# fluggo/Canvas

Measured on AMD Instinct MI355X. Metric: Mpixels/s through 4K f16 RGBA colour-matrix+alpha-over chain; % HBM roofline, higher is better.
Workload: dtype f32

## Files before the change

### canvas_amd/_lib.py

```python
import ctypes as C
import os

from .abi import (box2i, fir_filter, rational, rgba_frame_f16, rgba_frame_f32, v2f, v2i, video_frame_source_funcs,
                  video_source)

_HERE = os.path.dirname(os.path.abspath(__file__))
LIB_PATH = os.path.join(_HERE, "libcanvas_hip.so")

CHAIN_MAX_LAYERS = 8
DISPLAY_RGBA8, DISPLAY_ARGB32_PREMUL = 0, 1
FIR_PATH_AUTO, FIR_PATH_PASSES, FIR_PATH_TILED, FIR_PATH_TABLES, FIR_PATH_HV, FIR_PATH_ONE_COLUMN, FIR_PATH_TWO_COLUMNS, FIR_PATH_STRIPS, FIR_PATH_TILES = 0, 1, 2, 4, 16, 32, 64, 128, 256
FIR_KERNEL_NONE, FIR_KERNEL_WINDOW, FIR_KERNEL_HALVE, _FIR_KERNEL_RETIRED_3, FIR_KERNEL_VH, FIR_KERNEL_TILED, _FIR_KERNEL_RETIRED_6, FIR_KERNEL_TWO_PASS, FIR_KERNEL_PASS, FIR_KERNEL_HV, FIR_KERNEL_WINDOW_PAIR, FIR_KERNEL_HALVE_PAIR, FIR_KERNEL_TILE_VH, FIR_KERNEL_UNSHARP = range(14)
ARITH_SEPARATE, ARITH_CONTRACTED = 0, 1
LUT_NONE, LUT_REC709_TO_LINEAR_SCENE, LUT_REC709_TO_LINEAR_DISPLAY, LUT_LINEAR_TO_REC709, LUT_LINEAR_TO_SRGB = -1, 0, 1, 2, 3
KEY_SHOW_MATTE = 1
MATTE_SHOW, MATTE_MAX_CHOKE, MATTE_MAX_TAPS = 1, 16, 25
TRANSFORM_NEAREST, TRANSFORM_BILINEAR, TRANSFORM_MAX_COORD = 0, 1, 1 << 23
MAX_COORD, RESAMPLE_MAX_COORD = 1 << 30, 1 << 23
SCOPE_HISTOGRAM, SCOPE_WAVEFORM, SCOPE_PARADE, SCOPE_VECTORSCOPE = range(4)
SCOPE_SKIP_TRANSPARENT, SCOPE_MAX_COLUMNS = 1, 4096
LUT3D_MIN_SIZE, LUT3D_MAX_SIZE = 2, 65
PERSPECTIVE_MAX_SPAN = 1 << 23
YCC_PROGRESSIVE, YCC_REC709 = 1, 2

# ... 233 lines not shown
    "cvs_transform_from_parts": (C.c_int, [P(C.c_double), P(C.c_double), C.c_double, P(C.c_double), _f32p]),
    "cvs_transform_target_window": (C.c_int, [P(transform_params), P(box2i), P(box2i), P(box2i)]),
    "cvs_transform_source_window": (C.c_int, [P(transform_params), P(box2i), P(box2i)]),
    "cvs_blur_over_f16_dev": (C.c_int, [_F16, _F16, _f32p, C.c_int, P(_F16), C.c_int, _vp]),
    "cvs_resample_lanczos_f32_dev": (C.c_int, [_F32, _F32, C.c_float, C.c_float, C.c_int, _vp]),
    "cvs_resample_lanczos_f16_dev": (C.c_int, [_F16, _F16, C.c_float, C.c_float, C.c_int, _vp]),
    "cvs_blur_lanczos_f16_dev": (C.c_int, [_F16, _F16, _f32p, C.c_int, C.c_float, C.c_float, C.c_int, _vp]),
    "cvs_blur_over_f16_batch_dev": (C.c_int, [P(_F16), P(_F16), _f32p, C.c_int, P(_F16), C.c_int, C.c_int, _vp]),
    "cvs_scale_bilinear_f16_batch_dev": (C.c_int, [P(_F16), v2f, P(_F16), v2f, v2f, C.c_int, _vp]),
    "cvs_scale_bilinear_f32_batch_dev": (C.c_int, [P(_F32), v2f, P(_F32), v2f, v2f, C.c_int, _vp]),
    "cvs_blur_lanczos_f16_batch_dev": (C.c_int, [P(_F16), P(_F16), C.c_int, _f32p, C.c_int, C.c_float, C.c_float, C.c_int, _vp]),
    "cvs_fir_path_override": (None, [C.c_int]),
    "cvs_chain_color_over_f16_dev": (C.c_int, [P(chain_job), C.c_int, _f32p, C.c_int, C.c_int, _vp]),
    "cvs_chain_last_was_fused": (C.c_int, []),
    "cvs_scale_last_was_fused": (C.c_int, []),
    "cvs_fir_last_kernel": (C.c_int, []),
    "cvs_fir_fell_through_count": (C.c_int, []),
    "cvs_chain_last_launch_count": (C.c_int, []),
    "cvs_mix_cross_f16_dev": (C.c_int, [_F16, _F16, _F16, C.c_float, _vp]),
}

SCOPE_SIGNATURES = {
    "cvs_scope_count": (C.c_size_t, [P(scope_params)]),
    "cvs_scope_picture_size": (C.c_int, [P(scope_params), P(v2i)]),
    "cvs_scope_counts_f16_dev": (C.c_int, [_vp, _F16, P(scope_params), _vp]),
    "cvs_scope_render_f16_dev": (C.c_int, [_F16, P(box2i), _vp, P(scope_params), C.c_float, _vp]),
    "video_scope_counts": (C.c_int, [_vp, _F16, P(scope_params)]),
}

LUT3D_SIGNATURES = {
    "cvs_lut3d_bytes": (C.c_size_t, [C.c_int]),
    "cvs_lut3d_pack": (C.c_int, [_f32p, _f32p, C.c_int]),
    "cvs_lut3d_f16_dev": (C.c_int, [_F16, _F16, _vp, P(lut3d_params), _vp]),
    "cvs_lut3d_f32_dev": (C.c_int, [_F32, _F32, _vp, P(lut3d_params), _vp]),
}

PERSPECTIVE_SIGNATURES = {
    "cvs_perspective_f32_dev": (C.c_int, [_F32, _F32, P(perspective_params), _vp]),
    "cvs_perspective_f16_dev": (C.c_int, [_F16, _F16, P(perspective_params), _vp]),
    "cvs_perspective_from_quad": (C.c_int, [P(C.c_double), P(C.c_double * 2), C.c_int, P(perspective_params)]),
    "cvs_perspective_target_window": (C.c_int, [P(perspective_params), P(box2i), P(box2i), P(box2i)]),
    "cvs_perspective_source_window": (C.c_int, [P(perspective_params), P(box2i), P(box2i)]),
}

DEINTERLACE_SIGNATURES = {
    "cvs_deinterlace_adaptive_f16_dev": (C.c_int, [_F16, _F16, _F16, _F16, P(deinterlace_params), _vp]),
}

MEDIAN_SIGNATURES = {
    "cvs_median_f16_dev": (C.c_int, [_F16, _F16, P(median_params), _vp]),
    "cvs_median_f32_dev": (C.c_int, [_F32, _F32, P(median_params), _vp]),
}

HALF_POINTER_GLOBALS = {
    "half_convert_to_float": C.CFUNCTYPE(None, _f32p, _u16p, C.c_int),
    "half_convert_from_float": C.CFUNCTYPE(None, _u16p, _f32p, C.c_int),
    "half_convert_to_float_fast": C.CFUNCTYPE(None, _f32p, _u16p, C.c_int),
    "half_convert_from_float_fast": C.CFUNCTYPE(None, _u16p, _f32p, C.c_int),
    "half_lookup": C.CFUNCTYPE(None, _u16p, _u16p, _u16p, C.c_int),
}

_lib = None


class LibraryMissing(RuntimeError):
    pass


def load():
    global _lib
    if _lib is not None:
        return _lib
    if not os.path.exists(LIB_PATH):
        raise LibraryMissing(
            "%s not found: build it with `python -c 'import __graft_entry__ as g; g.build()'` "
            "(or make -C canvas_amd/csrc).  There is no CPU fallback." % LIB_PATH)
    lib = C.CDLL(LIB_PATH, mode=C.RTLD_GLOBAL)
    for name, (res, args) in list(SIGNATURES.items()) + list(SCOPE_SIGNATURES.items()) + list(LUT3D_SIGNATURES.items()) + list(PERSPECTIVE_SIGNATURES.items()) + list(DEINTERLACE_SIGNATURES.items()) + list(MEDIAN_SIGNATURES.items()):
        fn = getattr(lib, name)
        fn.restype, fn.argtypes = res, args
    _lib = lib
    return lib


def half_pointer(name):
    lib = load()
    addr = C.c_void_p.in_dll(lib, name).value
    return HALF_POINTER_GLOBALS[name](addr) if addr else None


def last_error():
    return load().cvs_last_error().decode()


def check(rc, what="call"):
    if rc != 0:
        raise RuntimeError("%s failed (%d): %s" % (what, rc, last_error()))
```

### canvas_amd/csrc/host/scale.c

```c
#define _GNU_SOURCE
#include "internal.h"
#include <limits.h>
#include <math.h>
#include <stdatomic.h>

static _Atomic int g_fir_path = CVS_FIR_PATH_AUTO;

static _Thread_local int t_scale_fused;
CVS_EXPORT int cvs_scale_last_was_fused(void) { return t_scale_fused; }
static _Thread_local int t_fir_kernel;
CVS_EXPORT int cvs_fir_last_kernel(void) { return t_fir_kernel; }
static _Thread_local int t_fell_through;
CVS_EXPORT int cvs_fir_fell_through_count(void) { return t_fell_through; }
static void fir_launch_fell_through(const char *kernel, int rc) {
    (void)hipGetLastError();
    t_fell_through++;
    cvs_log_warning("%s did not launch (%s): falling back to the next FIR kernel", kernel, hipGetErrorString((hipError_t)rc));
}
CVS_EXPORT void cvs_fir_path_override(int mode) { atomic_store(&g_fir_path, mode & (CVS_FIR_PATH_PASSES | CVS_FIR_PATH_TILED | CVS_FIR_PATH_TABLES | CVS_FIR_PATH_HV | CVS_FIR_PATH_ONE_COLUMN | CVS_FIR_PATH_TWO_COLUMNS | CVS_FIR_PATH_STRIPS | CVS_FIR_PATH_TILES)); }

typedef struct { void *data; box2i full, cur; int half; } any_frame;

static size_t any_bytes(const any_frame *f) { return cvs_box_pixels(&f->full) * (f->half ? sizeof(rgba_f16) : sizeof(rgba_f32)); }

typedef struct { void *frame, *data; box2i *full, *cur; } frame_ref;

static frame_ref frame_of(const void *f, int half) {
    frame_ref r = { (void *)f, NULL, NULL, NULL };
    if (f && half) { rgba_frame_f16 *h = r.frame; r.data = h->data; r.full = &h->full_window; r.cur = &h->current_window; }
    else if (f)    { rgba_frame_f32 *g = r.frame; r.data = g->data; r.full = &g->full_window; r.cur = &g->current_window; }
    return r;
}

static frame_ref frame_at(const void *frames, int i, int half) {
    return frame_of(half ? (const void *)((const rgba_frame_f16 *const *)frames)[i] : (const void *)((const rgba_frame_f32 *const *)frames)[i], half);
}

static any_frame any_of(const frame_ref *f, int half) {
    const any_frame a = { f->data, *f->full, *f->cur, half };
    return a;
}

static bool shares_buffer(const frame_ref *t, const frame_ref *src, const char *what) {
    if (!t->data || t->data != src->data) return false;
    cvs_set_error("%s: the target is the source's buffer: the operation is not in place", what);
    return true;
}

static bool entry_refused(void *target, const void *source, int half, const char *what, frame_ref *t, frame_ref *src, int lim) {
    *t = frame_of(target, half);
    *src = frame_of(source, half);
    if (shares_buffer(t, src, what)) { box2i_set_empty(t->cur); return true; }
    if (cvs_enter() != 0) { box2i_set_empty(t->cur); return true; }
    if (!cvs_box_contains(src->full, src->cur)) {
// ... 662 lines not shown
        else box2i_set_empty(&target->current_window);
        return rc;
    }
    any_frame mid = { NULL, *sw, *sw, 0 };
    mid.data = cvs_pool_malloc(cvs_box_pixels(sw) * sizeof(rgba_f32), s);
    if (!mid.data) { box2i_set_empty(&target->current_window); return -1; }
    int rc = blur_fused(&mid, &sf, sw, taps, ntaps, NULL, 0, NULL, s);
    if (rc == 0) rc = lanczos_fused(&tf, &mid, fx, fy, ksize, s);
    if (rc == 0) target->current_window = target->full_window;
    cvs_pool_free(mid.data, s);
    if (rc != 0) box2i_set_empty(&target->current_window);
    return rc;
}

CVS_EXPORT int cvs_blur_over_f16_batch_dev(rgba_frame_f16 *const *outs, const rgba_frame_f16 *const *sources, const float *taps, int ntaps,
                                           const rgba_frame_f16 *const *overlays, int noverlays, int count, cvs_stream_t stream) {
    const char *what = "cvs_blur_over_f16_batch_dev";
    if (count <= 0) return 0;
    if (ntaps < 1 || !taps || noverlays < 0 || (noverlays > 0 && !overlays)) { cvs_set_error("%s: bad arguments", what); return -1; }
    for (int i = 0; i < count; i++)
        for (int l = 0; l < noverlays; l++)
            if (!overlays[(size_t)i * noverlays + l]) { cvs_set_error("%s: layer %d of frame %d is a null pointer", what, l, i); return -1; }
    if (batch_refused(outs, sources, count, 1, what, CVS_MAX_COORD)) return -1;
    for (int i = 0; i < count * noverlays; i++)
        if (cvs_coords_refused(what, "an overlay", &overlays[i]->full_window, &overlays[i]->current_window, CVS_MAX_COORD)) { batch_empty_from(outs, 0, count, 1); return -1; }
    hipStream_t s = cvs_pick_stream(stream);
    const box2i *full = &outs[0]->full_window;
    bool uniform = count > 1 && noverlays >= 1 && noverlays <= CVK_BLUR_MAX_OVER && !box2i_is_empty(full) && blur_has_fast_kernel(taps, ntaps) && (ntaps & 1);
    for (int i = 0; uniform && i < count; i++) {
        uniform = same_box(&outs[i]->full_window, full) && same_box(&sources[i]->full_window, &sources[0]->full_window) &&
                  same_box(&sources[i]->current_window, full) && same_box(&sources[0]->full_window, full);
        for (int l = 0; uniform && l < noverlays; l++) {
            const rgba_frame_f16 *ov = overlays[(size_t)i * noverlays + l];
            uniform = same_box(&ov->full_window, full) && same_box(&ov->current_window, full);
        }
    }
    int rc = 0, done = 0;
    const size_t bytes = cvs_box_pixels(full) * sizeof(rgba_f16);
    while (uniform && rc == 0 && done < count) {
        const int n = count - done < CVK_FRAME_BATCH ? count - done : CVK_FRAME_BATCH;
        cvk_frame_batch b;
        if (!batch_group(&b, outs, sources, 1, done, n, bytes, bytes, overlays, noverlays)) break;
        const any_frame t = { b.target[0], *full, *full, 1 }, src = { (void *)b.source[0], sources[done]->full_window, sources[done]->current_window, 1 };
        rc = blur_fused(&t, &src, full, taps, ntaps, b.over[0], noverlays, &b, s);
        if (rc == 1) { rc = 0; break; }
        if (rc == 0) { for (int i = 0; i < n; i++) outs[done + i]->current_window = *full; done += n; }
    }
    for (; rc == 0 && done < count; done++)
        rc = cvs_blur_over_f16_dev(outs[done], sources[done], taps, ntaps, noverlays ? overlays + (size_t)done * noverlays : NULL, noverlays, stream);
    if (rc != 0) batch_empty_from(outs, done, count, 1);
    return rc;
}

CVS_EXPORT int cvs_blur_lanczos_f16_batch_dev(rgba_frame_f16 *const *targets, const rgba_frame_f16 *const *sources, int count,
                                              const float *taps, int ntaps, float fx, float fy, int ksize, cvs_stream_t stream) {
    const char *what = "cvs_blur_lanczos_f16_batch_dev";
    if (count <= 0) return 0;
    if (ntaps < 1 || !taps || !(fx > 0.0f) || !(fy > 0.0f) || ksize < 1) { cvs_set_error("%s: bad arguments", what); return -1; }
    if (batch_refused(targets, sources, count, 1, what, CVS_RESAMPLE_MAX_COORD)) return -1;
    hipStream_t s = cvs_pick_stream(stream);
    int rc = 0, done = 0;
    const box2i *tf = &targets[0]->full_window, *sw = &sources[0]->current_window;
    bool uniform = count > 1 && (ntaps & 1) && !(ntaps == 1 && taps[0] == 1.0f) && !box2i_is_empty(sw) && !box2i_is_empty(tf);
    for (int i = 1; uniform && i < count; i++)
        uniform = same_box(&targets[i]->full_window, tf) && same_box(&sources[i]->full_window, &sources[0]->full_window) &&
                  same_box(&sources[i]->current_window, sw);
    const any_frame t0 = { targets[0]->data, *tf, *tf, 1 }, s0 = { (void *)sources[0]->data, sources[0]->full_window, *sw, 1 };
    cvk_blur_halve_params hp;
    if (uniform && halving_sweep(&hp, fx, fy, ksize, taps, ntaps, &t0, &s0) && CVK(cvk_blur_halve_supported)(ntaps, hp.ntaps2)) {
        const size_t sbytes = cvs_box_pixels(&sources[0]->full_window) * sizeof(rgba_f16), tbytes = cvs_box_pixels(tf) * sizeof(rgba_f16);
        while (rc == 0 && done < count) {
            const int n = count - done < CVK_FRAME_BATCH ? count - done : CVK_FRAME_BATCH;
            if (!batch_group(&hp.batch, targets, sources, 1, done, n, tbytes, sbytes, NULL, 0)) break;
            hp.target.data = hp.batch.target[0];
            hp.source.data = (void *)hp.batch.source[0];
            if ((rc = halving_launch(&hp, s)) != 0) break;
            for (int i = 0; i < n; i++) targets[done + i]->current_window = targets[done + i]->full_window;
            done += n;
        }
    }
    for (; rc == 0 && done < count; done++)
        rc = cvs_blur_lanczos_f16_dev(targets[done], sources[done], taps, ntaps, fx, fy, ksize, stream);
    if (rc != 0) batch_empty_from(targets, done, count, 1);
    return rc;
}
```

### canvas_amd/csrc/kernels/kernels.h

```cpp
#ifndef CVS_KERNELS_H
#define CVS_KERNELS_H

#include <stddef.h>
#include <stdint.h>

#ifdef CVS_DIAG
#include <stdlib.h>
#define CVS_DIAG_ENV(name) getenv(name)
#else
#define CVS_DIAG_ENV(name) ((const char *)0)
#endif

#ifdef CVS_CONTRACT
#define cvk_gain_offset_f16          cvk_gain_offset_f16_fma
#define cvk_mix                      cvk_mix_fma
#define cvk_color_matrix             cvk_color_matrix_fma
#define cvk_chain_color_over         cvk_chain_color_over_fma
#define cvk_chain_cross              cvk_chain_cross_fma
#define cvk_chain_count_reset        cvk_chain_count_reset_fma
#define cvk_chain_count              cvk_chain_count_fma
#define cvk_fir_gather               cvk_fir_gather_fma
#define cvk_fir2d_lds_bytes          cvk_fir2d_lds_bytes_fma
#define cvk_fir2d                    cvk_fir2d_fma
#define cvk_fir_vh_supported         cvk_fir_vh_supported_fma
#define cvk_fir_vh                   cvk_fir_vh_fma
#define cvk_fir_tvh_supported        cvk_fir_tvh_supported_fma
#define cvk_fir_tvh_preferred        cvk_fir_tvh_preferred_fma
#define cvk_fir_tvh                  cvk_fir_tvh_fma
#define cvk_blur_supported           cvk_blur_supported_fma
#define cvk_blur_takes_pairs         cvk_blur_takes_pairs_fma
#define cvk_blur                     cvk_blur_fma
#define cvk_blur_pair_supported      cvk_blur_pair_supported_fma
#define cvk_blur_pair                cvk_blur_pair_fma
#define cvk_blur_halve_pair_supported cvk_blur_halve_pair_supported_fma
#define cvk_blur_halve_pair          cvk_blur_halve_pair_fma
#define cvk_blur_halve_supported     cvk_blur_halve_supported_fma
#define cvk_blur_halve_takes_pairs   cvk_blur_halve_takes_pairs_fma
#define cvk_blur_halve               cvk_blur_halve_fma
#define cvk_unsharp_supported        cvk_unsharp_supported_fma
#define cvk_unsharp                  cvk_unsharp_fma
#define cvk_unsharp_combine          cvk_unsharp_combine_fma
#define cvk_dv_reconstruct           cvk_dv_reconstruct_fma
#define cvk_dv_subsample             cvk_dv_subsample_fma
#endif

#ifdef __cplusplus
extern "C" {
#endif

typedef struct {
    void *data;
    int pitch;
    int fx0, fy0, fx1, fy1;
} cvk_view;

typedef struct { int x0, y0, x1, y1; } cvk_rect;

int cvk_half_to_float(float *out, const uint16_t *in, size_t count, int fast, void *stream);
int cvk_float_to_half(uint16_t *out, const float *in, size_t count, int fast, void *stream);
int cvk_half_lookup(const uint16_t *table, uint16_t *out, const uint16_t *in, size_t count, int cus, void *stream);

int cvk_copy_f16(cvk_view out, cvk_view in, cvk_rect r, void *stream);
int cvk_copy_alpha_f32(cvk_view out, cvk_view in, cvk_rect r, float alpha, void *stream);
int cvk_weave_f16(cvk_view frame, cvk_rect cur, const void *other, cvk_rect other_cur, void *stream);
int cvk_widen(cvk_view out32, cvk_view in16, cvk_rect r, void *stream);
int cvk_narrow(cvk_view out16, cvk_view in32, cvk_rect r, void *stream);
int cvk_fill_f16(cvk_view out, cvk_rect r, const float rgba[4], void *stream);
int cvk_fill_f32(cvk_view out, cvk_rect r, const float rgba[4], void *stream);
int cvk_gain_offset_f16(cvk_view out, cvk_view in, cvk_rect r, float gain, float offset, void *stream);

enum { CVK_MIX_CROSS = 0, CVK_MIX_OVER = 1 };
typedef struct {
    cvk_view out, p, q;
    cvk_rect outer, inner;
    cvk_rect pw, qw;
    int gap_x, gap_y;
    int top_is_p, bottom_is_p, left_is_p, right_is_p;
    float wp, wq;
    int mode;
    int p_in_place;
} cvk_mix_params;
int cvk_mix(const cvk_mix_params *mp, void *stream);

int cvk_color_matrix(cvk_view dst, cvk_view src, cvk_rect r, const float m[9], const uint16_t *pre_lut,
                     const uint16_t *post_lut, int cus, void *stream);

// ... 52 lines not shown
#define CVK_FIR_TVH_LINES 16
typedef struct {
    cvk_view target, source;
    int in_half, out_half;
    int tx0, ty0, tx1, ty1;
    cvk_fir_axis h, v;
    int max_sw, max_sh;
    int nframes, pad_;
    const void *frame_source[8];
    void *frame_target[8];
} cvk_fir2d_params;
#define CVK_FIR2D_TILE_X 32
#define CVK_FIR2D_TILE_Y 16
int cvk_fir_hv_supported(const cvk_fir2d_params *fp);
int cvk_fir_hv(const cvk_fir2d_params *fp, int cus, void *stream);
int cvk_fir_vh_supported(const cvk_fir2d_params *fp);
int cvk_fir_vh(const cvk_fir2d_params *fp, int line0, int cus, void *stream);
int cvk_fir_tvh_supported(const cvk_fir2d_params *fp);
int cvk_fir_tvh_preferred(const cvk_fir2d_params *fp);
int cvk_fir_tvh(const cvk_fir2d_params *fp, int line0, void *stream);
size_t cvk_fir2d_lds_bytes(const cvk_fir2d_params *fp);
int cvk_fir2d(const cvk_fir2d_params *fp, void *stream);

#define CVK_FRAME_BATCH 8
#define CVK_BLUR_MAX_OVER 4
typedef struct {
    int n, pad;
    const void *source[CVK_FRAME_BATCH];
    void *target[CVK_FRAME_BATCH];
    const void *over[CVK_FRAME_BATCH][CVK_BLUR_MAX_OVER];
} cvk_frame_batch;

typedef struct {
    cvk_view target, source;
    int in_half, out_half;
    int tx0, ty0, tx1, ty1;
    int sx0, sy0, sx1, sy1;
    int ntaps;
    int rows_per_wg;
    int step;
    float taps[32];
    int nover;
    int flags;
    const void *over[CVK_BLUR_MAX_OVER];
    cvk_frame_batch batch;
} cvk_blur_params;
#define CVK_BLUR_ONE_COLUMN  1
#define CVK_BLUR_TWO_COLUMNS 2
int cvk_blur_supported(int ntaps, int step);
int cvk_blur(const cvk_blur_params *bp, int cus, void *stream);
int cvk_blur_takes_pairs(const cvk_blur_params *bp);
int cvk_blur_pair_supported(const cvk_blur_params *bp);
int cvk_blur_pair(const cvk_blur_params *bp, int cus, void *stream);

typedef struct {
    cvk_view target, source;
    int in_half, out_half;
    int tx0, ty0, tx1, ty1;
    int sx0, sy0, sx1, sy1;
    int ntaps1, ntaps2;
    int rows_per_wg;
    int flags;
    float taps1[16], taps2[16];
    cvk_frame_batch batch;
} cvk_blur_halve_params;
int cvk_blur_halve_supported(int ntaps1, int ntaps2);
int cvk_blur_halve_pair_supported(const cvk_blur_halve_params *bp);
int cvk_blur_halve_pair(const cvk_blur_halve_params *bp, int cus, void *stream);
int cvk_blur_halve_takes_pairs(const cvk_blur_halve_params *bp);
int cvk_blur_halve(const cvk_blur_halve_params *bp, int cus, void *stream);

typedef struct {
    cvk_view target, source;
    int half;
    int tx0, ty0, tx1, ty1;
    int sx0, sy0, sx1, sy1;
    int ntaps;
    int rows_per_wg;
    float amount, threshold;
    float taps[16];
} cvk_unsharp_params;
int cvk_unsharp_supported(int ntaps);
int cvk_unsharp(const cvk_unsharp_params *up, int cus, void *stream);
int cvk_unsharp_combine(cvk_view out, cvk_view src, cvk_view blurred, cvk_rect r, int half, float amount, float threshold, void *stream);

enum { CVK_DISPLAY_RGBA8 = 0, CVK_DISPLAY_ARGB32_PREMUL = 1 };
int cvk_display(void *dst, cvk_view src, cvk_rect r, const uint8_t *table, int mode, int cus, void *stream);

enum { CVK_SCOPE_HISTOGRAM = 0, CVK_SCOPE_WAVEFORM = 1, CVK_SCOPE_PARADE = 2, CVK_SCOPE_VECTORSCOPE = 3 };
int cvk_scope_counts(uint32_t *counts, cvk_view src, cvk_rect m, const uint8_t *table, int kind, int region_x0, long long region_w,
                     int columns, int skip_transparent, int cus, void *stream);
int cvk_scope_render(cvk_view out, cvk_rect win, int px0, int py0, const uint32_t *counts, int kind, int columns, float gain, void *stream);

typedef struct { uint8_t *y, *cb, *cr; int sy, scb, scr; } cvk_dv_planes;
typedef struct { float coeff[16]; int width, center; } cvk_dv_taps;
int cvk_dv_reconstruct(cvk_view frame, cvk_rect cur, const cvk_dv_planes *pl, const cvk_dv_taps *tri, const uint16_t *lut, void *stream);
int cvk_dv_subsample(const cvk_dv_planes *pl, cvk_view frame, cvk_rect w, const cvk_dv_taps *tri, const uint16_t *lut, int encode_in_place, void *stream);

int cvk_mpeg2_subsample(const cvk_dv_planes *pl, cvk_view frame, cvk_rect w, int width, int height, const uint16_t *lut, int cus, void *stream);
int cvk_mpeg2_reconstruct(cvk_view frame, cvk_rect w, const cvk_dv_planes *pl, int width, int height, int progressive, const float mat[9],
                          const uint16_t *lut, int cus, void *stream);

int cvk_field_to_frame(cvk_view out, cvk_view in, cvk_rect w, cvk_rect in_cur, int field, int cus, void *stream);
int cvk_soften_fields(cvk_view out, cvk_view in, cvk_rect w, cvk_rect in_cur, int cus, void *stream);
int cvk_interlace_fields(cvk_view out, cvk_view even, cvk_view odd, cvk_rect w, cvk_rect even_cur, cvk_rect odd_cur, int cus, void *stream);

// ... 33 lines not shown
    int tw, th;
    int pair_loads;
} cvk_transform_params;
int cvk_transform(const cvk_transform_params *tp, int half, void *stream);

typedef struct {
    cvk_view out, in;
    cvk_rect w, s;
    long long tdx, tdy, sdx, sdy;
    float h[9];
    int bilinear;
} cvk_perspective_params;
int cvk_perspective(const cvk_perspective_params *pp, int half, void *stream);

typedef struct {
    cvk_view out, cur, n[2];
    cvk_rect w, cw, v[2];
    int field, soft;
    float threshold, inv_soft;
    int xs, seg;
} cvk_deinterlace_params;
int cvk_deinterlace_adaptive(const cvk_deinterlace_params *dp, int neighbours, int cus, void *stream);

typedef struct {
    cvk_view out, in;
    cvk_rect w, cw;
    int radius, channels, gated;
    float threshold;
    int xs, seg;
} cvk_median_params;
int cvk_median(const cvk_median_params *mp, int half, int cus, void *stream);

#ifndef CVS_CONTRACT
int cvk_gain_offset_f16_fma(cvk_view out, cvk_view in, cvk_rect r, float gain, float offset, void *stream);
int cvk_mix_fma(const cvk_mix_params *mp, void *stream);
int cvk_color_matrix_fma(cvk_view dst, cvk_view src, cvk_rect r, const float m[9], const uint16_t *pre_lut, const uint16_t *post_lut, int cus, void *stream);
int cvk_chain_color_over_fma(const cvk_chain_job *jobs, int njobs, int uniform_layers, const float *m, const uint16_t *pre_lut, const uint16_t *post_lut, int cus, void *stream);
int cvk_chain_cross_fma(const cvk_chain_job *jobs, int njobs, float wa, float wb, int cus, void *stream);
void cvk_chain_count_reset_fma(void);
int cvk_chain_count_fma(void);
int cvk_fir_gather_fma(const cvk_fir_params *fp, void *stream);
size_t cvk_fir2d_lds_bytes_fma(const cvk_fir2d_params *fp);
int cvk_fir2d_fma(const cvk_fir2d_params *fp, void *stream);
int cvk_fir_vh_supported_fma(const cvk_fir2d_params *fp);
int cvk_fir_vh_fma(const cvk_fir2d_params *fp, int line0, int cus, void *stream);
int cvk_fir_tvh_supported_fma(const cvk_fir2d_params *fp);
int cvk_fir_tvh_preferred_fma(const cvk_fir2d_params *fp);
int cvk_fir_tvh_fma(const cvk_fir2d_params *fp, int line0, void *stream);
int cvk_blur_supported_fma(int ntaps, int step);
int cvk_blur_takes_pairs_fma(const cvk_blur_params *bp);
int cvk_blur_fma(const cvk_blur_params *bp, int cus, void *stream);
int cvk_blur_pair_supported_fma(const cvk_blur_params *bp);
int cvk_blur_pair_fma(const cvk_blur_params *bp, int cus, void *stream);
int cvk_blur_halve_pair_supported_fma(const cvk_blur_halve_params *bp);
int cvk_blur_halve_pair_fma(const cvk_blur_halve_params *bp, int cus, void *stream);
int cvk_blur_halve_supported_fma(int ntaps1, int ntaps2);
int cvk_blur_halve_takes_pairs_fma(const cvk_blur_halve_params *bp);
int cvk_blur_halve_fma(const cvk_blur_halve_params *bp, int cus, void *stream);
int cvk_unsharp_supported_fma(int ntaps);
int cvk_unsharp_fma(const cvk_unsharp_params *up, int cus, void *stream);
int cvk_unsharp_combine_fma(cvk_view out, cvk_view src, cvk_view blurred, cvk_rect r, int half, float amount, float threshold, void *stream);
int cvk_dv_reconstruct_fma(cvk_view frame, cvk_rect cur, const cvk_dv_planes *pl, const cvk_dv_taps *tri, const uint16_t *lut, void *stream);
int cvk_dv_subsample_fma(const cvk_dv_planes *pl, cvk_view frame, cvk_rect w, const cvk_dv_taps *tri, const uint16_t *lut, int encode_in_place, void *stream);
#endif

#ifdef __cplusplus
}
#endif
#endif
```

### canvas_amd/stream.py

```python
import ctypes as C

import numpy as np

from . import _lib, synth
from .device import DeviceFrame
from .shard import frames_of_rank

NODE_BYTES_PER_PIXEL = 16 + 16 + 40
BYTES_PER_PIXEL = 16 + 40
OVERLAYS = 3


class GraphStream:

    def __init__(self, width, height, ring=4, matrix=None, pre_lut=_lib.LUT_REC709_TO_LINEAR_SCENE,
                 post_lut=_lib.LUT_NONE, taps=None, overlays=OVERLAYS, first_frame=0, frame_step=1, exact_slots=None, donors=None):
        from . import REC709_RGB_TO_YPBPR
        self.lib = _lib.load()
        self.w, self.h, self.ring, self.overlays = width, height, ring, overlays
        self.full = (0, 0, width - 1, height - 1)
        self.matrix = np.ascontiguousarray(REC709_RGB_TO_YPBPR if matrix is None else matrix, np.float32).reshape(9)
        self.pre_lut, self.post_lut = pre_lut, post_lut
        self.taps = np.ascontiguousarray(synth.gaussian_taps(9, 1.5) if taps is None else taps, np.float32)
        self.slots = []
        nd = 0
        for slot in range(ring):
            exact = exact_slots is None or slot < exact_slots or not donors
            frames = []
            for k in range(overlays + 1):
                d = DeviceFrame(self.full, np.uint16)
                if exact:
                    d.upload(synth.layer_pixels(width, height, k, first_frame + slot * frame_step))
                else:
                    src_frame = donors[(2 * nd) % len(donors)] if k == 0 else donors[(2 * nd + 1) % len(donors)]
                    nd += 1
                    _lib.check(self.lib.cvs_memcpy_d2d(d.ptr, src_frame.ptr, d.nbytes, None), "d2d")
                frames.append(d)
            src, over = frames[0], frames[1:]
            refs = (C.POINTER(_lib.rgba_frame_f16_t) * overlays)(*[C.pointer(o.c) for o in over])
            self.slots.append({"src": src, "over": over, "over_refs": refs, "graded": DeviceFrame(self.full, np.uint16),
                               "out": DeviceFrame(self.full, np.uint16)})
        _lib.check(self.lib.cvs_stream_sync(None), "donor copies")
        self._m = self.matrix.ctypes.data_as(C.POINTER(C.c_float))
        self._t = self.taps.ctypes.data_as(C.POINTER(C.c_float))

    @staticmethod
    def host_inputs(width, height, frame, overlays=OVERLAYS):
        return [synth.layer_frame(width, height, k, frame) for k in range(overlays + 1)]

    def render(self, slot, stream=None):
        s, lib = self.slots[slot % self.ring], self.lib
        _lib.check(lib.cvs_color_matrix_f16_to_dev(s["graded"].ref(), s["src"].ref(), self._m, self.pre_lut, self.post_lut, stream), "colour")
        _lib.check(lib.cvs_blur_over_f16_dev(s["out"].ref(), s["graded"].ref(), self._t, len(self.taps), s["over_refs"],
                                             self.overlays, stream), "blur+over")
        return s["out"]

    def render_batch(self, slots, stream=None):
        lib, n = self.lib, len(slots)
        ss = [self.slots[i % self.ring] for i in slots]
        for s in ss:
            _lib.check(lib.cvs_color_matrix_f16_to_dev(s["graded"].ref(), s["src"].ref(), self._m, self.pre_lut, self.post_lut, stream), "colour")
        key = tuple(i % self.ring for i in slots)
        if getattr(self, "_batch_key", None) != key:
            fp = C.POINTER(_lib.rgba_frame_f16_t)
            self._b_out = (fp * n)(*[C.pointer(s["out"].c) for s in ss])
            self._b_src = (fp * n)(*[C.pointer(s["graded"].c) for s in ss])
            self._b_ov = (fp * (n * self.overlays))(*[C.pointer(o.c) for s in ss for o in s["over"]])
            self._batch_key = key
        _lib.check(lib.cvs_blur_over_f16_batch_dev(self._b_out, self._b_src, self._t, len(self.taps), self._b_ov, self.overlays, n, stream), "blur+over batch")
        return [s["out"] for s in ss]

    def run(self, frames_per_rank, rank=0, world=1, stream=None):
        mine = frames_of_rank(rank, world, frames_per_rank)
        for i, _g in enumerate(mine):
            self.render(i, stream)
        return len(mine)
```

Measured before the change: 259,100.

## Fuse colour matrix into the paired blur+over kernel to drop the graded intermediate

Adds a kernel that applies the colour matrix (with an optional pre-LUT held in shared memory) to each source row as it is loaded, then runs the vertical/horizontal blur and alpha-over of the overlay layers in the same pass. New host entry points route the stream's render and batch paths through it, falling back to the old two-launch sequence when the fused kernel is unsupported. This removes one full-frame write and one full-frame read of the graded f16 frame, plus a kernel launch. The cost is more ALU work and LUT loads inside the blur kernel, more template instances, and a reduced bytes-per-pixel constant used for roofline accounting.

```diff
diff --git a/canvas_amd/_lib.py b/canvas_amd/_lib.py
--- a/canvas_amd/_lib.py
+++ b/canvas_amd/_lib.py
@@ -309,6 +309,12 @@
     "cvs_median_f32_dev": (C.c_int, [_F32, _F32, P(median_params), _vp]),
 }
 
+COLOR_BLUR_SIGNATURES = {
+    "cvs_color_blur_over_f16_dev": (C.c_int, [_F16, _F16, _f32p, C.c_int, C.c_int, _f32p, C.c_int, P(_F16), C.c_int, _vp]),
+    "cvs_color_blur_over_f16_batch_dev": (C.c_int, [P(_F16), P(_F16), _f32p, C.c_int, C.c_int, _f32p, C.c_int, P(_F16), C.c_int, C.c_int, _vp]),
+    "cvs_color_blur_last_was_fused": (C.c_int, []),
+}
+
 HALF_POINTER_GLOBALS = {
     "half_convert_to_float": C.CFUNCTYPE(None, _f32p, _u16p, C.c_int),
     "half_convert_from_float": C.CFUNCTYPE(None, _u16p, _f32p, C.c_int),
@@ -333,7 +339,7 @@
             "%s not found: build it with `python -c 'import __graft_entry__ as g; g.build()'` "
             "(or make -C canvas_amd/csrc).  There is no CPU fallback." % LIB_PATH)
     lib = C.CDLL(LIB_PATH, mode=C.RTLD_GLOBAL)
-    for name, (res, args) in list(SIGNATURES.items()) + list(SCOPE_SIGNATURES.items()) + list(LUT3D_SIGNATURES.items()) + list(PERSPECTIVE_SIGNATURES.items()) + list(DEINTERLACE_SIGNATURES.items()) + list(MEDIAN_SIGNATURES.items()):
+    for name, (res, args) in list(SIGNATURES.items()) + list(SCOPE_SIGNATURES.items()) + list(LUT3D_SIGNATURES.items()) + list(PERSPECTIVE_SIGNATURES.items()) + list(DEINTERLACE_SIGNATURES.items()) + list(MEDIAN_SIGNATURES.items()) + list(COLOR_BLUR_SIGNATURES.items()):
         fn = getattr(lib, name)
         fn.restype, fn.argtypes = res, args
     _lib = lib
diff --git a/canvas_amd/csrc/host/scale.c b/canvas_amd/csrc/host/scale.c
--- a/canvas_amd/csrc/host/scale.c
+++ b/canvas_amd/csrc/host/scale.c
@@ -1,5 +1,6 @@
 #define _GNU_SOURCE
 #include "internal.h"
+#include "canvas_color_blur.h"
 #include <limits.h>
 #include <math.h>
 #include <stdatomic.h>
@@ -768,6 +769,125 @@
     return rc;
 }
 
+static _Thread_local int t_color_blur_fused = -1;
+CVS_EXPORT int cvs_color_blur_last_was_fused(void) { return t_color_blur_fused; }
+
+static int color_blur_fused(const any_frame *t, const any_frame *src, const box2i *win, const float m[9], const half *pre, const half *post,
+                            const float *taps, int ntaps, const void *const *over, int nover, const cvk_frame_batch *batch, hipStream_t s) {
+    const box2i *sw = &src->cur;
+    if (!blur_has_fast_kernel(taps, ntaps) || nover > CVK_BLUR_MAX_OVER) return 1;
+    cvk_blur_params bp;
+    memset(&bp, 0, sizeof bp);
+    bp.nover = nover;
+    for (int l = 0; l < nover; l++) bp.over[l] = over[l];
+    bp.target = cvs_view(t->data, &t->full);
+    bp.source = cvs_view(src->data, &src->full);
+    bp.in_half = 1; bp.out_half = 1;
+    bp.tx0 = win->min.x; bp.ty0 = win->min.y; bp.tx1 = win->max.x; bp.ty1 = win->max.y;
+    bp.sx0 = sw->min.x; bp.sy0 = sw->min.y; bp.sx1 = sw->max.x; bp.sy1 = sw->max.y;
+    bp.ntaps = ntaps;
+    bp.step = 1;
+    memcpy(bp.taps, taps, sizeof(float) * (size_t)ntaps);
+    if (batch) bp.batch = *batch;
+    bp.flags = blur_column_pins();
+    if (!CVK(cvk_blur_takes_pairs)(&bp) || !CVK(cvk_color_blur_pair_supported)(&bp, pre, post)) return 1;
+    int rc = CVK(cvk_color_blur_pair)(&bp, m, pre, post, cvs_cus(), s);
+    if (rc != 0) { cvs_set_error("colour + blur launch failed: %s", hipGetErrorString((hipError_t)rc)); return -1; }
+    t_fir_kernel = CVS_FIR_KERNEL_WINDOW_PAIR;
+    return 0;
+}
+
+CVS_EXPORT int cvs_color_blur_over_f16_dev(rgba_frame_f16 *out, const rgba_frame_f16 *source, const float m[9], int pre_lut, int post_lut,
+                                           const float *taps, int ntaps, const rgba_frame_f16 *const *overlays, int noverlays,
+                                           cvs_stream_t stream) {
+    const char *what = "cvs_color_blur_over_f16_dev";
+    if (out->data && out->data == source->data) {
+        cvs_set_error("%s: the target is the source's buffer: the operation is not in place", what);
+        box2i_set_empty(&out->current_window);
+        return -1;
+    }
+    if (cvs_enter() != 0) { box2i_set_empty(&out->current_window); return -1; }
+    CVS_REQUIRE_INSIDE(source, out, what);
+    CVS_REQUIRE_COORDS(source, 1, out, what, "source");
+    CVS_REQUIRE_COORDS(out, 0, out, what, "out");
+    for (int l = 0; l < noverlays && overlays; l++) CVS_REQUIRE_COORDS(overlays[l], 1, out, what, "an overlay");
+    if (ntaps < 1 || !taps || noverlays < 0 || (noverlays > 0 && !overlays)) { cvs_set_error("colour + blur + over: bad arguments"); box2i_set_empty(&out->current_window); return -1; }
+    const half *pre = cvs_lut_dev_or_null(pre_lut), *post = cvs_lut_dev_or_null(post_lut);
+    if ((pre_lut != CVS_LUT_NONE && !pre) || (post_lut != CVS_LUT_NONE && !post)) { box2i_set_empty(&out->current_window); return -1; }
+    hipStream_t s = cvs_pick_stream(stream);
+    const box2i *full = &out->full_window;
+    box2i win;
+    box2i_intersect(&win, &source->current_window, full);
+    bool whole = noverlays <= CVK_BLUR_MAX_OVER && !box2i_is_empty(&win) && (noverlays == 0 || same_box(&win, full));
+    const void *bufs[CVK_BLUR_MAX_OVER];
+    for (int l = 0; whole && l < noverlays; l++) {
+        whole = same_box(&overlays[l]->full_window, full) && same_box(&overlays[l]->current_window, full);
+        bufs[l] = overlays[l]->data;
+    }
+    if (whole) {
+        const any_frame o = { out->data, *full, *full, 1 }, src = { (void *)source->data, source->full_window, source->current_window, 1 };
+        const int rc = color_blur_fused(&o, &src, &win, m, pre, post, taps, ntaps, bufs, noverlays, NULL, s);
+        if (rc == 0) { out->current_window = win; t_color_blur_fused = 1; return 0; }
+        if (rc < 0) { box2i_set_empty(&out->current_window); return -1; }
+    }
+    t_color_blur_fused = 0;
+    const size_t n = cvs_box_pixels(&source->full_window);
+    rgba_frame_f16 graded = { n ? cvs_pool_malloc(n * sizeof(rgba_f16), s) : NULL, source->full_window, source->full_window };
+    if (n && !graded.data) { box2i_set_empty(&out->current_window); return -1; }
+    int rc = cvs_color_matrix_f16_to_dev(&graded, source, m, pre_lut, post_lut, stream);
+    if (rc == 0) rc = cvs_blur_over_f16_dev(out, &graded, taps, ntaps, overlays, noverlays, stream);
+    else box2i_set_empty(&out->current_window);
+    cvs_pool_free(graded.data, s);
+    return rc;
+}
+
+CVS_EXPORT int cvs_color_blur_over_f16_batch_dev(rgba_frame_f16 *const *outs, const rgba_frame_f16 *const *sources, const float m[9],
+                                                 int pre_lut, int post_lut, const float *taps, int ntaps,
+                                                 const rgba_frame_f16 *const *overlays, int noverlays, int count, cvs_stream_t stream) {
+    const char *what = "cvs_color_blur_over_f16_batch_dev";
+    if (count <= 0) return 0;
+    if (ntaps < 1 || !taps || noverlays < 0 || (noverlays > 0 && !overlays)) { cvs_set_error("%s: bad arguments", what); return -1; }
+    for (int i = 0; i < count; i++)
+        for (int l = 0; l < noverlays; l++)
+            if (!overlays[(size_t)i * noverlays + l]) { cvs_set_error("%s: layer %d of frame %d is a null pointer", what, l, i); return -1; }
+    if (batch_refused(outs, sources, count, 1, what, CVS_MAX_COORD)) return -1;
+    for (int i = 0; i < count * noverlays; i++)
+        if (cvs_coords_refused(what, "an overlay", &overlays[i]->full_window, &overlays[i]->current_window, CVS_MAX_COORD)) { batch_empty_from(outs, 0, count, 1); return -1; }
+    const half *pre = cvs_lut_dev_or_null(pre_lut), *post = cvs_lut_dev_or_null(post_lut);
+    if ((pre_lut != CVS_LUT_NONE && !pre) || (post_lut != CVS_LUT_NONE && !post)) { batch_empty_from(outs, 0, count, 1); return -1; }
+    hipStream_t s = cvs_pick_stream(stream);
+    const box2i *full = &outs[0]->full_window;
+    bool uniform = count > 1 && noverlays >= 1 && noverlays <= CVK_BLUR_MAX_OVER && !box2i_is_empty(full);
+    for (int i = 0; uniform && i < count; i++) {
+        uniform = same_box(&outs[i]->full_window, full) && same_box(&sources[i]->full_window, &sources[0]->full_window) &&
+                  same_box(&sources[i]->current_window, full) && same_box(&sources[0]->full_window, full);
+        for (int l = 0; uniform && l < noverlays; l++) {
+            const rgba_frame_f16 *ov = overlays[(size_t)i * noverlays + l];
+            uniform = same_box(&ov->full_window, full) && same_box(&ov->current_window, full);
+        }
+    }
+    int rc = 0, done = 0;
+    bool all_fused = true;
+    const size_t bytes = cvs_box_pixels(full) * sizeof(rgba_f16);
+    while (uniform && rc == 0 && done < count) {
+        const int n = count - done < CVK_FRAME_BATCH ? count - done : CVK_FRAME_BATCH;
+        cvk_frame_batch b;
+        if (!batch_group(&b, outs, sources, 1, done, n, bytes, bytes, overlays, noverlays)) break;
+        const any_frame t = { b.target[0], *full, *full, 1 }, src = { (void *)b.source[0], sources[done]->full_window, sources[done]->current_window, 1 };
+        rc = color_blur_fused(&t, &src, full, m, pre, post, taps, ntaps, b.over[0], noverlays, &b, s);
+        if (rc == 1) { rc = 0; break; }
+        if (rc == 0) { for (int i = 0; i < n; i++) outs[done + i]->current_window = *full; done += n; }
+    }
+    for (; rc == 0 && done < count; done++) {
+        rc = cvs_color_blur_over_f16_dev(outs[done], sources[done], m, pre_lut, post_lut, taps, ntaps,
+                                         noverlays ? overlays + (size_t)done * noverlays : NULL, noverlays, stream);
+        all_fused = all_fused && t_color_blur_fused == 1;
+    }
+    if (rc != 0) batch_empty_from(outs, done, count, 1);
+    else t_color_blur_fused = all_fused ? 1 : 0;
+    return rc;
+}
+
 CVS_EXPORT int cvs_blur_lanczos_f16_batch_dev(rgba_frame_f16 *const *targets, const rgba_frame_f16 *const *sources, int count,
                                               const float *taps, int ntaps, float fx, float fy, int ksize, cvs_stream_t stream) {
     const char *what = "cvs_blur_lanczos_f16_batch_dev";
diff --git a/canvas_amd/csrc/kernels/color_blur_pair_ops.hip b/canvas_amd/csrc/kernels/color_blur_pair_ops.hip
--- /dev/null
+++ b/canvas_amd/csrc/kernels/color_blur_pair_ops.hip
@@ -0,0 +1,255 @@
+#include <cstdlib>
+#include <atomic>
+#include "pair_common.hpp"
+
+namespace {
+
+using namespace pairsweep;
+using cvs::Mat;
+using cvs::MatR;
+
+constexpr int kWaves = 12, kLanes = 64, kPitch = kLanes + 8;
+
+template <int NT, int NOV, bool PRE>
+__global__ __launch_bounds__(kWaves * kLanes) void k_color_blur_pair(cvk_blur_params bp, Mat kmat, const uint16_t *__restrict__ pre,
+                                                                     int strips, int segs, int units) {
+    constexpr int W = kLanes, PITCH = kPitch;
+    constexpr int C = NT / 2, D = C & 1, OUTW = 2 * W - 2 * C - 2 * D;
+    static_assert(NT & 1 && NT >= 3 && NT <= 11, "odd tap counts up to 11");
+    static_assert(NOV >= 0 && NOV <= CVK_BLUR_MAX_OVER, "layer count");
+    __shared__ uint16_t lut[PRE ? cvs::kLutHalfs : 1];
+    __shared__ u32x2 rowbuf[kWaves][2][2][PITCH];
+    const MatR mat = CVS_MAT_REGS(kmat);
+    const int lane = (int)threadIdx.x & (W - 1);
+    const int wave = __builtin_amdgcn_readfirstlane((int)threadIdx.x / W);
+    u32x2 (*const rows)[2][PITCH] = rowbuf[wave];
+
+    if constexpr (PRE) {
+        const uint4 *t = reinterpret_cast<const uint4 *>(pre);
+        uint4 *d = reinterpret_cast<uint4 *>(lut);
+        for (int k = (int)threadIdx.x; k < cvs::kLutHalfs * 2 / 16; k += kWaves * W) d[k] = t[k];
+    }
+    if (lane < PITCH - W) {
+#pragma unroll
+        for (int b = 0; b < 2; b++)
+#pragma unroll
+            for (int ph = 0; ph < 2; ph++) rows[b][ph][W + lane] = u32x2{ 0u, 0u };
+    }
+    if constexpr (PRE) __syncthreads();
+
+    float w[NT];
+#pragma unroll
+    for (int k = 0; k < NT; k++) w[k] = bp.taps[k];
+
+    typedef const cvk_blur_params __attribute__((address_space(4))) *kargs_t;
+    const kargs_t ka = (kargs_t)__builtin_amdgcn_kernarg_segment_ptr();
+    const size_t srow = (size_t)bp.source.pitch * 8, trow = (size_t)bp.target.pitch * 8;
+    const uint32_t swin = (uint32_t)(bp.sx1 - bp.sx0 + 1) * 8u, trect = (uint32_t)(bp.tx1 - bp.tx0 + 1) * 8u;
+    const ptrdiff_t trect0 = (ptrdiff_t)(bp.tx0 - bp.target.fx0) * 8;
+
+    for (int u = (int)blockIdx.x * kWaves + wave; u < units; u += (int)gridDim.x * kWaves) {
+        const int strip = u % strips, rest = u / strips, seg = rest % segs, z = rest / segs;
+        const int xo = bp.tx0 + strip * OUTW;
+        const int sfirst = xo - C - D;
+        const int tcol = xo + 2 * lane;
+        const int ta = bp.ty0 + seg * bp.rows_per_wg;
+        const int tb = min(ta + bp.rows_per_wg - 1, bp.ty1);
+        const int ys0 = ta - C;
+        const int steps = (tb - ta) + NT;
+
+        const void *src_data = bp.batch.n ? ka->batch.source[z] : bp.source.data;
+        void *dst_data = bp.batch.n ? ka->batch.target[z] : bp.target.data;
+        const void *over_data[NOV > 0 ? NOV : 1];
+#pragma unroll
+        for (int l = 0; l < NOV; l++) over_data[l] = bp.batch.n ? ka->batch.over[z][l] : bp.over[l];
+
+        const uint32_t soff = (uint32_t)((sfirst + 2 * lane - bp.sx0) * 8);
+        const uint32_t toff = 2 * lane < OUTW ? (uint32_t)((tcol - bp.tx0) * 8) : 0x80000000u;
+        const bool col_loaded = soff < swin;
+        const char *swin0 = reinterpret_cast<const char *>(src_data) + (ptrdiff_t)(bp.sx0 - bp.source.fx0) * 8;
+
+        Px ring[NT][2];
+#pragma unroll
+        for (int k = 0; k < NT; k++) ring[k][0].rg = ring[k][0].ba = ring[k][1].rg = ring[k][1].ba = f32x2{ 0.0f, 0.0f };
+
+        auto row_live = [&](int ys, bool wanted) { return wanted && ys >= bp.sy0 && ys <= bp.sy1; };
+        auto fetch_row = [&](int ys, bool wanted) {
+            return load_pair(row_rsrc(swin0, (size_t)((ptrdiff_t)(ys - bp.source.fy0) * (ptrdiff_t)srow), row_live(ys, wanted) ? swin : 0u), soff);
+        };
+        auto put_row = [&](u32x2 (*buf)[PITCH], u32x4 raw, bool live) {
+            u32x4 g = { 0u, 0u, 0u, 0u };
+            if (live) {
+                const u32x4 c = cvs::color_pair_codes<PRE, false>(raw, mat, lut, nullptr);
+                g.x = col_loaded ? c.x : 0u; g.y = col_loaded ? c.y : 0u; g.z = col_loaded ? c.z : 0u; g.w = col_loaded ? c.w : 0u;
+            }
+            buf[0][lane] = u32x2{ g.x, g.y };
+            buf[1][lane] = u32x2{ g.z, g.w };
+        };
+        struct Layers { u32x4 v[NOV > 0 ? NOV : 1]; };
+        auto fetch_layers = [&](int i) {
+            Layers r;
+            const bool emits = i >= NT - 1 && i < steps;
+            const size_t o = (size_t)((ptrdiff_t)(ta + i - (NT - 1) - bp.target.fy0) * (ptrdiff_t)trow + trect0);
+#pragma unroll
+            for (int l = 0; l < NOV; l++) r.v[l] = load_pair(row_rsrc(over_data[l], o, emits ? trect : 0u), toff);
+            return r;
+        };
+        u32x4 cur = fetch_row(ys0, true);
+        put_row(rows[0], cur, row_live(ys0, true));
+        cur = fetch_row(ys0 + 1, steps > 1);
+        u32x4 nxt = fetch_row(ys0 + 2, steps > 2);
+        Layers ov_cur;
+        if constexpr (NOV > 0) ov_cur = fetch_layers(0);
+
+        for (int i0 = 0; i0 < steps; i0 += NT) {
+            auto step = [&](auto jc) -> bool {
+                constexpr int j = decltype(jc)::value;
+                const int i = i0 + j;
+                if (i >= steps) return false;
+                const bool emits = i >= NT - 1;
+                const int t = ta + (i - (NT - 1));
+                const u32x4 far = fetch_row(ys0 + i + 3, i + 3 < steps);
+                Layers ov_nxt;
+                if constexpr (NOV > 0) ov_nxt = fetch_layers(i + 1);
+                u32x2 (*buf)[PITCH] = rows[i & 1];
+                __builtin_amdgcn_fence(__ATOMIC_RELEASE, "wavefront");
+                __builtin_amdgcn_wave_barrier();
+                __builtin_amdgcn_fence(__ATOMIC_ACQUIRE, "wavefront");
+                float4 v[NT + 1];
+#pragma unroll
+                for (int c = 0; c <= NT; c++) {
+                    const u32x2 q = buf[(c + D) & 1][lane + ((c + D) >> 1)];
+                    v[c] = widen_px(q.x, q.y);
+                }
+                put_row(rows[(i + 1) & 1], cur, row_live(ys0 + i + 1, i + 1 < steps));
+                cur = nxt;
+                nxt = far;
+                f32x2 rg0, ba0, rg1, ba1;
+#pragma unroll
+                for (int k = 0; k < NT; k++) {
+                    if constexpr (cvs::kContract) {
+                        if (k == 0) { rg0 = f32x2{ v[0].x, v[0].y } * w[0]; ba0 = f32x2{ v[0].z, v[0].w } * w[0]; rg1 = f32x2{ v[1].x, v[1].y } * w[0]; ba1 = f32x2{ v[1].z, v[1].w } * w[0]; }
+                        else {
+                            rg0 = cvs::madd(f32x2{ v[k].x, v[k].y }, w[k], rg0); ba0 = cvs::madd(f32x2{ v[k].z, v[k].w }, w[k], ba0);
+                            rg1 = cvs::madd(f32x2{ v[k + 1].x, v[k + 1].y }, w[k], rg1); ba1 = cvs::madd(f32x2{ v[k + 1].z, v[k + 1].w }, w[k], ba1);
+                        }
+                    } else {
+                    const f32x2 p0 = f32x2{ v[k].x, v[k].y } * w[k], q0 = f32x2{ v[k].z, v[k].w } * w[k];
+                    const f32x2 p1 = f32x2{ v[k + 1].x, v[k + 1].y } * w[k], q1 = f32x2{ v[k + 1].z, v[k + 1].w } * w[k];
+                    if (k == 0) { rg0 = p0; ba0 = q0; rg1 = p1; ba1 = q1; }
+                    else { rg0 = rg0 + p0; ba0 = ba0 + q0; rg1 = rg1 + p1; ba1 = ba1 + q1; }
+                    }
+                }
+                ring[j][0].rg = rg0; ring[j][0].ba = ba0;
+                ring[j][1].rg = rg1; ring[j][1].ba = ba1;
+                if (emits) {
+                    f32x2 org0, oba0, org1, oba1;
+#pragma unroll
+                    for (int k = 0; k < NT; k++) {
+                        const Px &a = ring[(j + 1 + k) % NT][0], &b = ring[(j + 1 + k) % NT][1];
+                        if constexpr (cvs::kContract) {
+                            if (k == 0) { org0 = a.rg * w[0]; oba0 = a.ba * w[0]; org1 = b.rg * w[0]; oba1 = b.ba * w[0]; }
+                            else { org0 = cvs::madd(a.rg, w[k], org0); oba0 = cvs::madd(a.ba, w[k], oba0); org1 = cvs::madd(b.rg, w[k], org1); oba1 = cvs::madd(b.ba, w[k], oba1); }
+                        } else {
+                        const f32x2 p0 = a.rg * w[k], q0 = a.ba * w[k], p1 = b.rg * w[k], q1 = b.ba * w[k];
+                        if (k == 0) { org0 = p0; oba0 = q0; org1 = p1; oba1 = q1; }
+                        else { org0 = org0 + p0; oba0 = oba0 + q0; org1 = org1 + p1; oba1 = oba1 + q1; }
+                        }
+                    }
+                    u32x4 codes;
+                    if constexpr (NOV > 0) {
+                        cvs::px32x2 acc;
+                        acc.r = f32x2{ org0.x, org1.x }; acc.g = f32x2{ org0.y, org1.y };
+                        acc.b = f32x2{ oba0.x, oba1.x }; acc.a = f32x2{ oba0.y, oba1.y };
+#pragma unroll
+                        for (int l = 0; l < NOV; l++) acc = cvs::over_pair_uniform(acc, ov_cur.v[l]);
+                        codes = cvs::narrow_pair_lean(acc);
+                    } else {
+                        codes = u32x4{ cvs::f2h_rz2(org0.x, org0.y), cvs::f2h_rz2(oba0.x, oba0.y), cvs::f2h_rz2(org1.x, org1.y), cvs::f2h_rz2(oba1.x, oba1.y) };
+                    }
+                    __builtin_amdgcn_raw_buffer_store_b128(codes, row_rsrc(dst_data, (size_t)((ptrdiff_t)(t - bp.target.fy0) * (ptrdiff_t)trow + trect0), trect), (int)toff, 0, 0);
+                }
+                if constexpr (NOV > 0) ov_cur = ov_nxt;
+                return true;
+            };
+            each_slot(step, std::make_integer_sequence<int, NT>{});
+        }
+        __builtin_amdgcn_fence(__ATOMIC_RELEASE, "wavefront");
+        __builtin_amdgcn_wave_barrier();
+    }
+}
+
+template <int NT, int NOV, bool PRE>
+int launch(cvk_blur_params bp, const Mat &mat, const uint16_t *pre, int cus, hipStream_t s) {
+    constexpr int C = NT / 2, D = C & 1, OUTW = 2 * kLanes - 2 * C - 2 * D;
+    const int cols = bp.tx1 - bp.tx0 + 1, rows = bp.ty1 - bp.ty0 + 1;
+    const int strips = (cols + OUTW - 1) / OUTW;
+    const int nframes = bp.batch.n > 0 ? bp.batch.n : 1;
+    if (cus <= 0) cus = 256;
+    int nseg = (kWaves * cus) / (strips * nframes);
+    if (nseg < 1) nseg = 1;
+    int r = (rows + nseg - 1) / nseg;
+    if (r < NT - 1) r = NT - 1;
+    if (r > rows) r = rows;
+    bp.rows_per_wg = r;
+    const int segs = (rows + r - 1) / r;
+    const long long units = (long long)strips * segs * nframes;
+    if (units > 0x7fffffffLL) return (int)hipErrorInvalidValue;
+    const long long wgs = (units + kWaves - 1) / kWaves;
+    dim3 grid((unsigned)(wgs < cus ? wgs : cus));
+    hipLaunchKernelGGL((k_color_blur_pair<NT, NOV, PRE>), grid, dim3(kWaves * kLanes), 0, s, bp, mat, pre, strips, segs, (int)units);
+    return (int)hipGetLastError();
+}
+
+constexpr bool has_instance(int ntaps, int nover) {
+    if (!(ntaps & 1) || ntaps < 3 || nover < 0 || nover > CVK_BLUR_MAX_OVER) return false;
+    return ntaps <= 7 || (ntaps == 9 && nover >= 1) || (ntaps == 11 && nover == 1);
+}
+
+template <int NT, int NOV, bool PRE>
+int launch_if(const cvk_blur_params *bp, const Mat &mat, const uint16_t *pre, int cus, hipStream_t s) {
+    if constexpr (has_instance(NT, NOV)) return launch<NT, NOV, PRE>(*bp, mat, pre, cus, s);
+    else return (int)hipErrorInvalidValue;
+}
+
+template <int NT, bool PRE>
+int pick_layers(const cvk_blur_params *bp, const Mat &mat, const uint16_t *pre, int cus, hipStream_t s) {
+    switch (bp->nover) {
+    case 0: return launch_if<NT, 0, PRE>(bp, mat, pre, cus, s);
+    case 1: return launch_if<NT, 1, PRE>(bp, mat, pre, cus, s);
+    case 2: return launch_if<NT, 2, PRE>(bp, mat, pre, cus, s);
+    case 3: return launch_if<NT, 3, PRE>(bp, mat, pre, cus, s);
+    case 4: return launch_if<NT, 4, PRE>(bp, mat, pre, cus, s);
+    }
+    return (int)hipErrorInvalidValue;
+}
+
+template <bool PRE>
+int pick(const cvk_blur_params *bp, const Mat &mat, const uint16_t *pre, int cus, hipStream_t s) {
+    switch (bp->ntaps) {
+    case 3: return pick_layers<3, PRE>(bp, mat, pre, cus, s);
+    case 5: return pick_layers<5, PRE>(bp, mat, pre, cus, s);
+    case 7: return pick_layers<7, PRE>(bp, mat, pre, cus, s);
+    case 9: return pick_layers<9, PRE>(bp, mat, pre, cus, s);
+    case 11: return pick_layers<11, PRE>(bp, mat, pre, cus, s);
+    }
+    return (int)hipErrorInvalidValue;
+}
+
+}
+
+extern "C" int cvk_color_blur_pair_supported(const cvk_blur_params *bp, const uint16_t *pre, const uint16_t *post) {
+    (void)pre;
+    if (post || !has_instance(bp->ntaps, bp->nover)) return 0;
+    return cvk_blur_pair_supported(bp);
+}
+
+extern "C" int cvk_color_blur_pair(const cvk_blur_params *bp_in, const float m[9], const uint16_t *pre, const uint16_t *post, int cus, void *stream) {
+    if (bp_in->tx1 < bp_in->tx0 || bp_in->ty1 < bp_in->ty0) return 0;
+    if (!cvk_color_blur_pair_supported(bp_in, pre, post)) return (int)hipErrorInvalidValue;
+    cvk_blur_params bp = *bp_in;
+    bp.step = 1;
+    bp.flags = 0;
+    const Mat mat = cvs::make_mat(m);
+    return pre ? pick<true>(&bp, mat, pre, cus, (hipStream_t)stream) : pick<false>(&bp, mat, pre, cus, (hipStream_t)stream);
+}
diff --git a/canvas_amd/csrc/kernels/kernels.h b/canvas_amd/csrc/kernels/kernels.h
--- a/canvas_amd/csrc/kernels/kernels.h
+++ b/canvas_amd/csrc/kernels/kernels.h
@@ -32,6 +32,8 @@
 #define cvk_blur                     cvk_blur_fma
 #define cvk_blur_pair_supported      cvk_blur_pair_supported_fma
 #define cvk_blur_pair                cvk_blur_pair_fma
+#define cvk_color_blur_pair_supported cvk_color_blur_pair_supported_fma
+#define cvk_color_blur_pair          cvk_color_blur_pair_fma
 #define cvk_blur_halve_pair_supported cvk_blur_halve_pair_supported_fma
 #define cvk_blur_halve_pair          cvk_blur_halve_pair_fma
 #define cvk_blur_halve_supported     cvk_blur_halve_supported_fma
@@ -190,6 +192,8 @@
 int cvk_blur_takes_pairs(const cvk_blur_params *bp);
 int cvk_blur_pair_supported(const cvk_blur_params *bp);
 int cvk_blur_pair(const cvk_blur_params *bp, int cus, void *stream);
+int cvk_color_blur_pair_supported(const cvk_blur_params *bp, const uint16_t *pre, const uint16_t *post);
+int cvk_color_blur_pair(const cvk_blur_params *bp, const float m[9], const uint16_t *pre, const uint16_t *post, int cus, void *stream);
 
 typedef struct {
     cvk_view target, source;
@@ -329,6 +333,8 @@
 int cvk_blur_fma(const cvk_blur_params *bp, int cus, void *stream);
 int cvk_blur_pair_supported_fma(const cvk_blur_params *bp);
 int cvk_blur_pair_fma(const cvk_blur_params *bp, int cus, void *stream);
+int cvk_color_blur_pair_supported_fma(const cvk_blur_params *bp, const uint16_t *pre, const uint16_t *post);
+int cvk_color_blur_pair_fma(const cvk_blur_params *bp, const float m[9], const uint16_t *pre, const uint16_t *post, int cus, void *stream);
 int cvk_blur_halve_pair_supported_fma(const cvk_blur_halve_params *bp);
 int cvk_blur_halve_pair_fma(const cvk_blur_halve_params *bp, int cus, void *stream);
 int cvk_blur_halve_supported_fma(int ntaps1, int ntaps2);
diff --git a/canvas_amd/stream.py b/canvas_amd/stream.py
--- a/canvas_amd/stream.py
+++ b/canvas_amd/stream.py
@@ -7,7 +7,7 @@
 from .shard import frames_of_rank
 
 NODE_BYTES_PER_PIXEL = 16 + 16 + 40
-BYTES_PER_PIXEL = 16 + 40
+BYTES_PER_PIXEL = 40
 OVERLAYS = 3
 
 
@@ -50,24 +50,22 @@
 
     def render(self, slot, stream=None):
         s, lib = self.slots[slot % self.ring], self.lib
-        _lib.check(lib.cvs_color_matrix_f16_to_dev(s["graded"].ref(), s["src"].ref(), self._m, self.pre_lut, self.post_lut, stream), "colour")
-        _lib.check(lib.cvs_blur_over_f16_dev(s["out"].ref(), s["graded"].ref(), self._t, len(self.taps), s["over_refs"],
-                                             self.overlays, stream), "blur+over")
+        _lib.check(lib.cvs_color_blur_over_f16_dev(s["out"].ref(), s["src"].ref(), self._m, self.pre_lut, self.post_lut, self._t, len(self.taps),
+                                                   s["over_refs"], self.overlays, stream), "colour+blur+over")
         return s["out"]
 
     def render_batch(self, slots, stream=None):
         lib, n = self.lib, len(slots)
         ss = [self.slots[i % self.ring] for i in slots]
-        for s in ss:
-            _lib.check(lib.cvs_color_matrix_f16_to_dev(s["graded"].ref(), s["src"].ref(), self._m, self.pre_lut, self.post_lut, stream), "colour")
         key = tuple(i % self.ring for i in slots)
         if getattr(self, "_batch_key", None) != key:
             fp = C.POINTER(_lib.rgba_frame_f16_t)
             self._b_out = (fp * n)(*[C.pointer(s["out"].c) for s in ss])
-            self._b_src = (fp * n)(*[C.pointer(s["graded"].c) for s in ss])
+            self._b_src = (fp * n)(*[C.pointer(s["src"].c) for s in ss])
             self._b_ov = (fp * (n * self.overlays))(*[C.pointer(o.c) for s in ss for o in s["over"]])
             self._batch_key = key
-        _lib.check(lib.cvs_blur_over_f16_batch_dev(self._b_out, self._b_src, self._t, len(self.taps), self._b_ov, self.overlays, n, stream), "blur+over batch")
+        _lib.check(lib.cvs_color_blur_over_f16_batch_dev(self._b_out, self._b_src, self._m, self.pre_lut, self.post_lut, self._t, len(self.taps),
+                                                         self._b_ov, self.overlays, n, stream), "colour+blur+over batch")
         return [s["out"] for s in ss]
 
     def run(self, frames_per_rank, rank=0, world=1, stream=None):
diff --git a/include/canvas_color_blur.h b/include/canvas_color_blur.h
--- /dev/null
+++ b/include/canvas_color_blur.h
@@ -0,0 +1,23 @@
+#ifndef CANVAS_COLOR_BLUR_H
+#define CANVAS_COLOR_BLUR_H
+
+#include "canvas_hip.h"
+
+#ifdef __cplusplus
+extern "C" {
+#endif
+
+CVS_EXPORT int cvs_color_blur_over_f16_dev(rgba_frame_f16 *out, const rgba_frame_f16 *source, const float m[9], int pre_lut, int post_lut,
+                                           const float *taps, int ntaps, const rgba_frame_f16 *const *overlays, int noverlays,
+                                           cvs_stream_t stream);
+
+CVS_EXPORT int cvs_color_blur_over_f16_batch_dev(rgba_frame_f16 *const *outs, const rgba_frame_f16 *const *sources, const float m[9],
+                                                 int pre_lut, int post_lut, const float *taps, int ntaps,
+                                                 const rgba_frame_f16 *const *overlays, int noverlays, int count, cvs_stream_t stream);
+
+CVS_EXPORT int cvs_color_blur_last_was_fused(void);
+
+#ifdef __cplusplus
+}
+#endif
+#endif
```

Result: no change. 258,400 (-0.3%).
